# johannesulf/nautilus

Hardware: AMD Instinct MI355X
Metric: effective posterior samples/sec + |dlogZ| vs analytic, 50-dim Gaussian (higher is better)
Workload: dtype f64

## Files before the change

nautilus_amd/csrc/nb_eval_fast.hip:

```cpp
#include "nb_common.h"
#include "nb_launch.h"

#include <type_traits>

#include "nb_mlp.h"

namespace {

constexpr int FAST_MAX_GROUPS = 1024;

struct FastArgs {
  const double* blob;
  int sample;
  const nb_gd* x;
  const long long* idx;
  int m;
  int recentre;
  long long n;
  unsigned char* out_u8;
  double* out_f64;
  unsigned long long seed;
  unsigned long long offset;
  unsigned long long* counters;
  const FastGroup* groups;
  const int* totals;
  const int* dense;
  long long n_pad;
  int n_groups;
  int out_mode;
  unsigned char* st;
  int* first;
};

constexpr int FAST_B_DOUBLES =
    (NB_HT1 * NB_HT2 + NB_HT2 * NB_HT3 + NB_HT3) * NB_TILE;

typedef const void __attribute__((address_space(1))) * nbf_gptr;
typedef void __attribute__((address_space(3))) * nbf_lptr;

template <int DT, int T>
__device__ __forceinline__ void ell_eval_centre(
    const double* c, const double* tiles, int n_dim,
    const double (&xin)[T][4 * DT], int lane, int lg, double (&y)[T][4 * DT],
    double (&r2)[T]) {
  double d[T][4 * DT];
#pragma unroll
  for (int ks = 0; ks < 4 * DT; ++ks) {
    const double cv = c[4 * ks + lg];
#pragma unroll
    for (int t = 0; t < T; ++t) d[t][ks] = xin[t][ks] - cv;
  }
  double part[T];
#pragma unroll
  for (int t = 0; t < T; ++t) part[t] = 0.0;
  const int live = n_dim - 16 * (DT - 1);
  const bool small = DT > 1 && live >= 1 && live <= 4;
  const int lane4 = (lane >> 4) * 16 + (lane & 3);
#pragma unroll
  for (int ht = 0; ht < DT; ++ht) {
    if (ht == DT - 1 && small) {
      double r4[T];
#pragma unroll
      for (int t = 0; t < T; ++t) r4[t] = 0.0;
#pragma unroll
      for (int ks = 0; ks < 4 * (ht + 1) - 2; ++ks) {
        const int kt = ks >> 2, s = ks & 3;
        const double a =
            tiles[(ht * (ht + 1) / 2 + kt) * NB_TILE + s * 64 + lane4];
#pragma unroll
        for (int t = 0; t < T; ++t) r4[t] = MFMA4(a, d[t][ks], r4[t]);
      }
#pragma unroll
      for (int t = 0; t < T; ++t) {
        y[t][4 * ht] = r4[t];
        y[t][4 * ht + 1] = y[t][4 * ht + 2] = y[t][4 * ht + 3] = 0.0;
        part[t] += r4[t] * r4[t];
      }
    } else if (16 * ht < n_dim) {
      nb_d4 acc[T];
#pragma unroll
      for (int t = 0; t < T; ++t) acc[t] = nb_d4{0.0, 0.0, 0.0, 0.0};
#pragma unroll
      for (int ks = 0; ks < 4 * (ht + 1); ++ks) {
        const int kt = ks >> 2, s = ks & 3;
        const double a =
            tiles[(ht * (ht + 1) / 2 + kt) * NB_TILE + s * 64 + lane];
#pragma unroll
        for (int t = 0; t < T; ++t) acc[t] = MFMA(a, d[t][ks], acc[t]);
      }
#pragma unroll
      for (int t = 0; t < T; ++t)
#pragma unroll
        for (int r = 0; r < 4; ++r) {
          y[t][4 * ht + r] = acc[t][r];
          part[t] += acc[t][r] * acc[t][r];
        }
    } else {
#pragma unroll
      for (int t = 0; t < T; ++t)
#pragma unroll
        for (int r = 0; r < 4; ++r) y[t][4 * ht + r] = 0.0;
    }
  }
#pragma unroll
  for (int t = 0; t < T; ++t) r2[t] = lane_group_sum(part[t]);
}

template <int DT, int T>
__device__ __forceinline__ void load_points_raw(
    const nb_gd* __restrict__ x, const long long (&row_of)[T], int n_dim,
    int lane, double2 (&raw)[T][2 * DT]) {
  int lg = lane >> 4;
  asm volatile("" : "+v"(lg));
  asm volatile("" : "+s"(x));
  if ((n_dim & 1) == 0) {
#pragma unroll
    for (int t = 0; t < T; ++t) {
      const nb_gd* row = x + row_of[t] * n_dim;
#pragma unroll
      for (int j = 0; j < 2 * DT; ++j) {
        const int f = 8 * j + 2 * lg;
        raw[t][j] = *(const NB_G double2*)(row + (f < n_dim ? f : n_dim - 2));
      }
    }
  } else {
#pragma unroll
    for (int t = 0; t < T; ++t) {
      const nb_gd* row = x + row_of[t] * n_dim;
#pragma unroll
      for (int j = 0; j < 2 * DT; ++j) {
        const int f = 8 * j + 2 * lg;
        raw[t][j].x = row[f < n_dim ? f : n_dim - 1];
        raw[t][j].y = row[f + 1 < n_dim ? f + 1 : n_dim - 1];
      }
    }
  }
}

template <int DT, int T>
__device__ __forceinline__ void points_from_raw(
    const double2 (&raw)[T][2 * DT], const bool (&valid)[T], int n_dim,
    int lg, double (&xin)[T][4 * DT]) {
#pragma unroll
  for (int t = 0; t < T; ++t)
#pragma unroll
    for (int j = 0; j < 2 * DT; ++j) {
      const int f = 8 * j + 2 * lg;
      xin[t][2 * j] = (valid[t] && f < n_dim) ? raw[t][j].x : 0.0;
      xin[t][2 * j + 1] = (valid[t] && f + 1 < n_dim) ? raw[t][j].y : 0.0;
    }
}

constexpr int FAST_REGION = 38 * NB_TILE;

template <int DT, int KT1, bool BATCH>
__global__ void __launch_bounds__(512) nb_eval_fast_kernel(FastArgs a) {
  constexpr int T = 1, NW = 8, DP = 16 * DT;
  constexpr int KS1 = 4 * KT1;
  constexpr bool TWO = KT1 * NB_HT1 * NB_TILE > FAST_REGION;
  constexpr int KA = TWO ? (KT1 + 1) / 2 : KT1;
  constexpr int NT = DT * (DT + 1) / 2;
  constexpr int HEAD = 128;
  constexpr int TAIL = HEAD + NT * NB_TILE;
  constexpr int TC = (2 + 2 * DP + 127) / 128;
  constexpr int ELL_CHUNKS = 1 + 2 * NT + TC;
  static_assert(DP <= HEAD, "centre fits the head");
  static_assert(TAIL + TC * 128 <= FAST_REGION, "ellipsoid block fits a region");
  static_assert(KA * NB_HT1 * NB_TILE <= FAST_REGION, "layer-1 chunk fits");
  constexpr int NA_D = KA * NB_HT1 * NB_TILE;
  constexpr int NB1_D = (KT1 - KA) * NB_HT1 * NB_TILE;
  constexpr int NC_D = FAST_B_DOUBLES;
  extern __shared__ __attribute__((aligned(16))) double lds[];
  auto reg = [&](int i) __attribute__((always_inline)) {
    return lds + (i & 1) * FAST_REGION;
  };

  const int lane = threadIdx.x & 63;
  const int wave = __builtin_amdgcn_readfirstlane(threadIdx.x >> 6);
  const int lg = lane >> 4;
  const bool m_sample = a.sample != 0;
  const double* blob = a.blob;
  const int n_dim = (int)nb_hdr(blob, NB_H_NDIM);
  const int K = (int)nb_hdr(blob, NB_H_K);
  const bool use_cube = nb_hdr(blob, NB_H_USECUBE) != 0;
  const int ks1 = (n_dim + 1 + 3) >> 2;
  const long long net_stride = nb_hdr(blob, NB_H_NET_STRIDE);
  unsigned long long cnt_ell = 0, cnt_mlp = 0;
  long long sup = blockIdx.x;

  struct Pass {
    const double* nb;
    const double* shift;
    int E, b;
    long long base;
    int n_valid;
  };
  int* pp = (int*)(lds + 2 * FAST_REGION);
  long long n_super;
  if constexpr (BATCH) {
    if (wave == 0) {
      int run = 0;
      for (int g0 = 0; g0 < a.n_groups; g0 += 64) {
        const int g = g0 + lane;
        int v = g < a.n_groups ? (a.totals[g] + 127) >> 7 : 0;
#pragma unroll
        for (int d = 1; d < 64; d <<= 1) {
          const int u = __shfl_up(v, d);
          if (lane >= d) v += u;
        }
        if (g < a.n_groups) pp[g + 1] = run + v;
        run += __shfl(v, 63);
      }
      if (lane == 0) pp[0] = 0;
    }
    __syncthreads();
    n_super = pp[a.n_groups];
    if (sup >= n_super) return;
  } else {
    n_super = (a.n + 16 * NW * T - 1) / (16 * NW * T);
  }
  auto pass_of = [&](long long P) __attribute__((always_inline)) {
    Pass ps;
    if constexpr (BATCH) {
      const long long Pc = P < n_super ? P : n_super - 1;
      int lo = 0, hi = a.n_groups;
      while (hi - lo > 1) {
        const int mid = (lo + hi) >> 1;
        if (pp[mid] <= (int)Pc) lo = mid; else hi = mid;
      }
      const int g = __builtin_amdgcn_readfirstlane(lo);
      const FastGroup gd = a.groups[g];
      ps.nb = gd.nb;
      ps.shift = a.recentre != 0 ? gd.shift : nullptr;
      ps.E = gd.E;
      ps.b = gd.b;
      const int s0 = ((int)Pc - __builtin_amdgcn_readfirstlane(pp[g])) << 7;
      ps.base = (long long)g * a.n_pad + s0;
      const int left = a.totals[g] - s0;
      ps.n_valid = P < n_super ? (left < 128 ? left : 128) : 0;
    } else {
      ps.nb = blob + nb_hdr(blob, NB_H_OFF_NEURAL) +
              a.m * nb_hdr(blob, NB_H_NEURAL_STRIDE);
      ps.shift = (a.recentre != 0 && nb_hdr(blob, NB_H_OFF_SHIFT) != 0)
                     ? blob + nb_hdr(blob, NB_H_OFF_SHIFT) : nullptr;
      ps.E = (int)nb_hdr(blob, NB_H_E);
      ps.b = 0;
      ps.base = 0;
      ps.n_valid = 0;
    }
    return ps;
  };
  Pass cur_p = pass_of(sup);

  const double* dma_src = nullptr;
  double* dma_dst = nullptr;
  int dma_c = 0, dma_n = 0;
  bool dma_ell = false;
  auto dma_begin = [&](const double* src, double* dst, int n_doubles)
      __attribute__((always_inline)) {
    dma_src = src; dma_dst = dst; dma_c = wave; dma_n = n_doubles >> 7;
    dma_ell = false;
  };
  auto dma_begin_ell = [&](const double* nb_blk, double* dst)
      __attribute__((always_inline)) {
    dma_src = nb_blk; dma_dst = dst; dma_c = wave;
    dma_n = ELL_CHUNKS;
    dma_ell = true;
  };
  auto dma_one = [&]() __attribute__((always_inline)) {
    int s_off, d_off;
    if (!dma_ell) {
      s_off = d_off = dma_c * 128;
    } else if (dma_c < 1) {
      s_off = 2 + 2 * DP;
      d_off = 0;
    } else if (dma_c < 1 + 2 * NT) {
      const int p = (dma_c - 1) >> 1, half = (dma_c - 1) & 1;
      int ht = 0;
      while ((ht + 1) * (ht + 2) / 2 <= p) ++ht;
      const int kt = p - ht * (ht + 1) / 2;
      s_off = 2 + 3 * DP + (kt * DT + ht) * NB_TILE + half * 128;
      d_off = HEAD + p * NB_TILE + half * 128;
    } else {
      const int i = dma_c - 1 - 2 * NT;
      s_off = nb_ell_block_size(DT) + i * 128;
      d_off = TAIL + i * 128;
    }
    __builtin_amdgcn_global_load_lds(
        (nbf_gptr)(dma_src + s_off + 2 * lane),
        (nbf_lptr)(dma_dst + d_off), 16, 0, 0);
    dma_c += NW;
  };
  auto dma_tick = [&]() __attribute__((always_inline)) {
    if (dma_c < dma_n) dma_one();
  };
  auto dma_flush = [&]() __attribute__((always_inline)) {
    while (dma_c < dma_n) dma_one();
  };

  int q = 0;
  dma_begin_ell(cur_p.nb, reg(0));
  dma_flush();
  long long pt[T];
  bool valid[T];
  double2 xraw[T][2 * DT];
  auto row_of = [&](long long p) __attribute__((always_inline)) {
    return p < a.n ? (a.idx != nullptr ? a.idx[p] : p) : 0ll;
  };
  auto row_in = [&](const Pass& ps, int t) __attribute__((always_inline)) {
    const int slot = (wave * T + t) * 16 + (lane & 15);
    return (long long)a.dense[ps.base + (slot < ps.n_valid ? slot : 0)];
  };
  long long nrow[T];
#pragma unroll
  for (int t = 0; t < T; ++t) {
    pt[t] = ((sup * NW + wave) * T + t) * 16 + (lane & 15);
    valid[t] = pt[t] < a.n;
    if constexpr (BATCH) nrow[t] = row_in(cur_p, t);
    else nrow[t] = row_of(pt[t]);
  }
  load_points_raw<DT, T>(a.x, nrow, n_dim, lane, xraw);

  for (; sup < n_super; sup += gridDim.x) {
    const double* nb_m = cur_p.nb;
    const double* shift = cur_p.shift;
    const int E = cur_p.E;
    const double* nets = nb_m + nb_ell_block_size(DT) + 2 + 2 * DP;
    const Pass next_p = pass_of(sup + gridDim.x);
    int lgp = lg;
    asm volatile("" : "+v"(lgp));
    long long crow[T];
    dma_begin(nets, reg(q ^ 1), NA_D);
    dma_flush();
    asm volatile("s_waitcnt vmcnt(%0)" ::"n"((NA_D / 128 + NW - 1) / NW)
                 : "memory");
    __syncthreads();
    const double* blk = reg(q);
    const double thr = blk[TAIL];

    bool in_cube[T], acc_outer[T], want[T];
    double xin[T][4 * DT];
#pragma unroll
    for (int t = 0; t < T; ++t) {
      pt[t] = ((sup * NW + wave) * T + t) * 16 + (lane & 15);
      in_cube[t] = true;
      if constexpr (BATCH) {
        valid[t] = (wave * T + t) * 16 + (lane & 15) < cur_p.n_valid;
        crow[t] = nrow[t];
        nrow[t] = row_in(next_p, t);
      } else {
        valid[t] = pt[t] < a.n;
        nrow[t] = row_of((((sup + gridDim.x) * NW + wave) * T + t) * 16 +
                         (lane & 15));
      }
    }
    points_from_raw<DT, T>(xraw, valid, n_dim, lgp, xin);
    if (shift != nullptr) {
#pragma unroll
      for (int ks = 0; ks < 4 * DT; ++ks) {
        const double sv = shift[4 * ks + lgp];
        const bool on = shift[DP + 4 * ks + lgp] != 0.0;
#pragma unroll
        for (int t = 0; t < T; ++t) {
          const double v = xin[t][ks] + sv;
          xin[t][ks] = on ? v - floor(v) : xin[t][ks];
        }
      }
    }
    if (m_sample) {
      bool cbad[T];
#pragma unroll
      for (int t = 0; t < T; ++t) cbad[t] = false;
#pragma unroll
      for (int ks = 0; ks < 4 * DT; ++ks) {
        const int f = 8 * (ks >> 1) + 2 * lgp + (ks & 1);
        const bool boxed = use_cube && f < n_dim;
#pragma unroll
        for (int t = 0; t < T; ++t)
          cbad[t] |= boxed && !(xin[t][ks] >= 0.0 && xin[t][ks] < 1.0);
      }
#pragma unroll
      for (int t = 0; t < T; ++t) {
        in_cube[t] = !point_any(cbad[t], lane);
        acc_outer[t] = in_cube[t];
        want[t] = valid[t] && acc_outer[t];
      }
    } else {
#pragma unroll
      for (int t = 0; t < T; ++t) { acc_outer[t] = false; want[t] = valid[t]; }
    }

    double y[T][4 * DT], r2[T];
    bool box_bad[T], inside_e[T], need[T];
    ell_eval_centre<DT, T>(blk, blk + HEAD, n_dim, xin, lane, lgp, y, r2);
#pragma unroll
    for (int t = 0; t < T; ++t) box_bad[t] = false;
    bool wave_mlp = false;
#pragma unroll
    for (int t = 0; t < T; ++t) {
      inside_e[t] = !box_bad[t] && r2[t] < 1.0;
      need[t] = m_sample ? (want[t] && inside_e[t]) : valid[t];
      cnt_ell += __popcll(__ballot(want[t] && lg == 0));
      cnt_mlp += (unsigned long long)E * __popcll(__ballot(need[t] && lg == 0));
      wave_mlp |= need[t];
    }
    wave_mlp = __any(wave_mlp);

    double tin[T][KS1];
    {
      const double* r_mean = blk + TAIL + 2;
      const double* r_isc = r_mean + DP;
#pragma unroll
      for (int ks = 0; ks < KS1; ++ks) {
        const int f = 4 * ks + lgp;
        if (ks < 4 * DT) {
          const double mv = r_mean[f], sv = r_isc[f];
          const double pad = (f == n_dim) ? 1.0 : 0.0;
#pragma unroll
          for (int t = 0; t < T; ++t) {
            const double v = (y[t][ks] - mv) * sv;
            tin[t][ks] = (f < n_dim) ? v : pad;
          }
        } else {
#pragma unroll
          for (int t = 0; t < T; ++t) tin[t][ks] = (f == n_dim) ? 1.0 : 0.0;
        }
      }
    }
    asm volatile("s_waitcnt vmcnt(0)" ::: "memory");
    __syncthreads();
#pragma unroll
    for (int t = 0; t < T; ++t) asm volatile("" : "+v"(nrow[t]));

    double total[T];
#pragma unroll
    for (int t = 0; t < T; ++t) total[t] = 0.0;
    int cur = q ^ 1;

    auto stage_end = [&]() __attribute__((always_inline)) {
      dma_flush();
      asm volatile("s_waitcnt vmcnt(0)" ::: "memory");
      __syncthreads();
      cur ^= 1;
    };
    auto network = [&](int e, auto last_c) __attribute__((always_inline)) {
      constexpr bool LAST = decltype(last_c)::value;
      const double* w_e = nets + e * net_stride;
      double h1[T][4 * NB_HT1];
      if constexpr (TWO) {
        dma_begin(w_e + NA_D, reg(cur ^ 1), NB1_D);
        if (wave_mlp)
          fl_chunk<T, KS1, NB_HT1, 0, 4 * KA, 2>(reg(cur), ks1, tin, lane, h1,
                                                dma_tick);
        stage_end();
        dma_begin(w_e + NA_D + NB1_D, reg(cur ^ 1), NC_D);
        if (wave_mlp) {
          fl_chunk<T, KS1, NB_HT1, 4 * KA, KS1, 1>(reg(cur), ks1, tin, lane,
                                                  h1, dma_tick);
          fl_pad<T, NB_HT1, 25, 0>(h1, lane);
        }
        stage_end();
      } else {
        dma_begin(w_e + NA_D, reg(cur ^ 1), NC_D);
        if (wave_mlp) {
          fl_chunk<T, KS1, NB_HT1, 0, KS1, 1>(reg(cur), ks1, tin, lane, h1,
                                             dma_tick);
          fl_pad<T, NB_HT1, 25, 0>(h1, lane);
        }
        stage_end();
      }
      if constexpr (LAST) {
        load_points_raw<DT, T>(a.x, nrow, n_dim, lane, xraw);
        dma_begin_ell(next_p.nb, reg(cur ^ 1));
      } else {
        dma_begin(nets + (e + 1) * net_stride, reg(cur ^ 1), NA_D);
      }
      if (wave_mlp) {
        const double* w2 = reg(cur);
        const double* w3 = w2 + NB_HT1 * NB_HT2 * NB_TILE;
        const double* w4 = w3 + NB_HT2 * NB_HT3 * NB_TILE;
        double h2[T][4 * NB_HT2], h3[T][4 * NB_HT3], o[T][4];
        double a2[FlFirst<8, NB_HT2>::NA], a3[FlFirst<8, NB_HT3>::NA],
            a4[FlFirst<8, 1>::NA];
        fl_read_first<8, NB_HT2>(w2, lane, a2);
        fl_layer_from<T, 8, 26, 0, NB_HT2, true, 2, 1, 0>(
            w2, 26, h1, lane, h2, a2,
            [&]() __attribute__((always_inline)) {
              fl_read_first<8, NB_HT3>(w3, lane, a3);
            },
            dma_tick);
        fl_pad<T, NB_HT2, 12, 2>(h2, lane);
        fl_layer_from<T, 8, 13, 0, NB_HT3, true, 2, 2, 0>(
            w3, 13, h2, lane, h3, a3,
            [&]() __attribute__((always_inline)) {
              fl_read_first<8, 1>(w4, lane, a4);
            },
            dma_tick);
        fl_pad<T, NB_HT3, 5, 0>(h3, lane);
        fl_layer_from<T, 8, 6, 0, 1, true, 2, 5, 0>(
            w4, 6, h3, lane, o, a4, []() __attribute__((always_inline)) {},
            dma_tick);
#pragma unroll
        for (int t = 0; t < T; ++t) total[t] += o[t][0];
      }
      stage_end();
    };
    for (int e = 0; e + 1 < E; ++e) network(e, std::false_type{});
    network(E - 1, std::true_type{});
    q = cur;

#pragma unroll
    for (int t = 0; t < T; ++t) {
      const double score = __shfl(total[t], lane & 15) / (double)E;
      if constexpr (BATCH) {
        if (valid[t] && lg == 0 && score > thr) {
          a.st[crow[t]] = a.out_mode == 2 ? (unsigned char)3 : (unsigned char)2;
          if (a.out_mode == 1) atomicMin(&a.first[crow[t]], cur_p.b);
        }
      } else if (m_sample) {
        bool ok = inside_e[t];
        if (need[t]) ok = inside_e[t] && (score > thr);
        const unsigned char flags =
            (acc_outer[t] ? 1 : 0) | ((acc_outer[t] && ok) ? 2 : 0);
        if (valid[t] && lg == 0) a.out_u8[pt[t]] = flags;
      } else if (valid[t] && lg == 0) {
        a.out_f64[2 * pt[t]] = r2[t];
        a.out_f64[2 * pt[t] + 1] = score;
      }
    }
    cur_p = next_p;
  }
  if (a.counters != nullptr && lane == 0) {
    atomicAdd(&a.counters[1], cnt_ell);
    atomicAdd(&a.counters[2], cnt_mlp);
  }
}

template <int DT, int KT1, bool BATCH>
int launch_fast_impl(const FastArgs& a, hipStream_t stream) {
  const size_t lds = (size_t)2 * FAST_REGION * sizeof(double) +
                     (BATCH ? (FAST_MAX_GROUPS + 1) * sizeof(int) : 0);
  if (const int rc = nb_allow_lds<nb_eval_fast_kernel<DT, KT1, BATCH>>(lds))
    return rc;
  const long long n_super = (a.n + 127) / 128;
  long long blocks = n_super < 256 ? n_super : 256;
  hipLaunchKernelGGL((nb_eval_fast_kernel<DT, KT1, BATCH>),
                     dim3((unsigned)blocks), dim3(512), lds, stream, a);
  return NB_OK;
}

template <int DT, int KT1>
int launch_fast(const FastArgs& a, hipStream_t stream) {
  return a.groups != nullptr ? launch_fast_impl<DT, KT1, true>(a, stream)
                             : launch_fast_impl<DT, KT1, false>(a, stream);
}

}

bool nb_eval_fast_eligible(int n_dim, int K, int M, int E, bool sample) {
  if (n_dim > 128 || M < 1 || E < 1) return false;
  return !sample || (K <= 1 && M == 1);
}

static int dispatch_fast(const FastArgs& a, int n_dim, hipStream_t stream) {
  const int kt1 = (n_dim + 1 + 15) / 16;
  const int rc = nb_tile_dispatch((n_dim + 15) / 16, [&](auto dt) {
    constexpr int DT = decltype(dt)::value;
    return kt1 == DT ? launch_fast<DT, DT>(a, stream)
                     : launch_fast<DT, DT + 1>(a, stream);
  });
  if (rc != NB_OK) return rc;
  NB_HIP_CHECK(hipGetLastError());
  return NB_OK;
}

int nb_launch_eval_fast(const double* blob_dev, int n_dim, bool sample, int m,
                        int recentre, const double* x, const long long* idx,
                        long long n,
                        unsigned char* out_u8, double* out_f64,
                        unsigned long long seed, unsigned long long offset,
                        hipStream_t stream) {
  if (n <= 0) return NB_OK;
  FastArgs a = {};
  a.blob = blob_dev; a.sample = sample ? 1 : 0; a.x = (const nb_gd*)x; a.n = n;
  a.idx = idx; a.m = m; a.recentre = recentre;
  a.out_u8 = out_u8; a.out_f64 = out_f64; a.seed = seed; a.offset = offset;
  a.counters = nb_eval_counters();
  return dispatch_fast(a, n_dim, stream);
}

int nb_launch_eval_fast_batch(const double* blob0_dev, int n_dim, int recentre,
                              const double* x, const void* groups_dev,
                              int n_groups, const int* totals_dev,
                              const int* dense_dev, long long n_pad,
                              long long n_upper, int out_mode,
                              unsigned char* st, int* first,
                              hipStream_t stream) {
  if (n_upper <= 0 || n_groups <= 0) return NB_OK;
  if (n_groups > FAST_MAX_GROUPS) {
    nb_set_error("nb_launch_eval_fast_batch: %d groups (limit %d)", n_groups,
                 FAST_MAX_GROUPS);
    return NB_ERR_ARG;
  }
  FastArgs a = {};
  a.blob = blob0_dev; a.sample = 0; a.x = (const nb_gd*)x;
  a.n = n_upper + 128ll * n_groups;
  a.recentre = recentre;
  a.counters = nb_eval_counters();
  a.groups = (const FastGroup*)groups_dev; a.n_groups = n_groups;
  a.totals = totals_dev; a.dense = dense_dev; a.n_pad = n_pad;
  a.out_mode = out_mode; a.st = st; a.first = first;
  return dispatch_fast(a, n_dim, stream);
}
```

Before: 2.595 million.

## Keep ellipsoid block resident in LDS and reuse layer-1 region across iterations

For non-batched small-dimension configurations, the kernel now sizes LDS so the ellipsoid block lives in its own resident area, and the first-layer weights stay in a fixed region. This removes the per-iteration re-DMA of the ellipsoid block and the layer-1 chunk plus one barrier per super-iteration. Prologue and epilogue are factored into lambdas, and an optional compile-time stagger mode (off by default) lets half the waves precompute the next prologue. The catch is a larger LDS footprint, which may reduce occupancy, and more code complexity.

```diff
diff --git a/nautilus_amd/csrc/nb_eval_fast.hip b/nautilus_amd/csrc/nb_eval_fast.hip
--- a/nautilus_amd/csrc/nb_eval_fast.hip
+++ b/nautilus_amd/csrc/nb_eval_fast.hip
@@ -106,10 +106,11 @@
   for (int t = 0; t < T; ++t) r2[t] = lane_group_sum(part[t]);
 }
 
-template <int DT, int T>
+template <int DT, int T, int NR>
 __device__ __forceinline__ void load_points_raw(
     const nb_gd* __restrict__ x, const long long (&row_of)[T], int n_dim,
-    int lane, double2 (&raw)[T][2 * DT]) {
+    int lane, double2 (&raw)[T][NR]) {
+  static_assert(NR >= 2 * DT, "a row's slots fit");
   int lg = lane >> 4;
   asm volatile("" : "+v"(lg));
   asm volatile("" : "+s"(x));
@@ -137,9 +138,9 @@
   }
 }
 
-template <int DT, int T>
+template <int DT, int T, int NR>
 __device__ __forceinline__ void points_from_raw(
-    const double2 (&raw)[T][2 * DT], const bool (&valid)[T], int n_dim,
+    const double2 (&raw)[T][NR], const bool (&valid)[T], int n_dim,
     int lg, double (&xin)[T][4 * DT]) {
 #pragma unroll
   for (int t = 0; t < T; ++t)
@@ -152,12 +153,43 @@
 }
 
 constexpr int FAST_REGION = 38 * NB_TILE;
+constexpr size_t FAST_LDS_BUDGET = 160 * 1024;
+#ifndef NB_FAST_STAGGER
+#define NB_FAST_STAGGER 0
+#endif
+constexpr bool FAST_STAGGER = NB_FAST_STAGGER != 0;
+
+constexpr int fast_block_doubles(int DT) {
+  return 128 + DT * (DT + 1) / 2 * NB_TILE + (2 + 32 * DT + 127) / 128 * 128;
+}
+constexpr bool fast_two(int KT1) {
+  return KT1 * NB_HT1 * NB_TILE > FAST_REGION;
+}
+constexpr size_t fast_resident_bytes(int DT, int KT1) {
+  return ((size_t)(KT1 * NB_HT1 + 38) * NB_TILE + fast_block_doubles(DT)) *
+         sizeof(double);
+}
+constexpr bool fast_resident(int DT, int KT1, bool BATCH) {
+  return !BATCH && !fast_two(KT1) &&
+         fast_resident_bytes(DT, KT1) <= FAST_LDS_BUDGET;
+}
+constexpr size_t fast_lds_bytes(int DT, int KT1, bool BATCH) {
+  return fast_resident(DT, KT1, BATCH)
+             ? fast_resident_bytes(DT, KT1)
+             : (size_t)2 * FAST_REGION * sizeof(double) +
+                   (BATCH ? (FAST_MAX_GROUPS + 1) * sizeof(int) : 0);
+}
 
 template <int DT, int KT1, bool BATCH>
 __global__ void __launch_bounds__(512) nb_eval_fast_kernel(FastArgs a) {
   constexpr int T = 1, NW = 8, DP = 16 * DT;
   constexpr int KS1 = 4 * KT1;
-  constexpr bool TWO = KT1 * NB_HT1 * NB_TILE > FAST_REGION;
+  constexpr bool TWO = fast_two(KT1);
+  constexpr bool RES = fast_resident(DT, KT1, BATCH);
+  static_assert(fast_lds_bytes(DT, KT1, BATCH) <= FAST_LDS_BUDGET,
+                "regions, ellipsoid block and pass table fit the LDS");
+  static_assert(RES == (!BATCH && (DT <= 3 || (DT == 4 && KT1 == 4))),
+                "resident form: every DT <= 3 and <4, 4>");
   constexpr int KA = TWO ? (KT1 + 1) / 2 : KT1;
   constexpr int NT = DT * (DT + 1) / 2;
   constexpr int HEAD = 128;
@@ -165,15 +197,18 @@
   constexpr int TC = (2 + 2 * DP + 127) / 128;
   constexpr int ELL_CHUNKS = 1 + 2 * NT + TC;
   static_assert(DP <= HEAD, "centre fits the head");
+  static_assert(TAIL + TC * 128 == fast_block_doubles(DT), "block size");
   static_assert(TAIL + TC * 128 <= FAST_REGION, "ellipsoid block fits a region");
   static_assert(KA * NB_HT1 * NB_TILE <= FAST_REGION, "layer-1 chunk fits");
   constexpr int NA_D = KA * NB_HT1 * NB_TILE;
   constexpr int NB1_D = (KT1 - KA) * NB_HT1 * NB_TILE;
   constexpr int NC_D = FAST_B_DOUBLES;
   extern __shared__ __attribute__((aligned(16))) double lds[];
+  constexpr int REG0_D = RES ? KT1 * NB_HT1 * NB_TILE : FAST_REGION;
   auto reg = [&](int i) __attribute__((always_inline)) {
-    return lds + (i & 1) * FAST_REGION;
-  };
+    return lds + (i & 1) * REG0_D;
+  };
+  double* const blk_res = lds + REG0_D + FAST_REGION;
 
   const int lane = threadIdx.x & 63;
   const int wave = __builtin_amdgcn_readfirstlane(threadIdx.x >> 6);
@@ -298,12 +333,151 @@
     while (dma_c < dma_n) dma_one();
   };
 
+  constexpr int NR = RES ? 2 * KT1 : 2 * DT;
+  auto slot_of = [&](long long P, int t) __attribute__((always_inline)) {
+    int l = lane;
+    asm volatile("" : "+v"(l));
+    return ((P * NW + wave) * T + t) * 16 + (l & 15);
+  };
+  enum : unsigned { PS_VALID = 1, PS_OUTER = 2, PS_INSIDE = 4, PS_NEED = 8 };
+  struct PState {
+    unsigned bits[T];
+    bool wave_mlp;
+    double r2[T];
+  };
+  auto prologue = [&](const double* blk, const double* shift, int E,
+                      const double2 (&raw)[T][NR], const bool (&valid)[T],
+                      PState& s, double (&tin)[T][KS1])
+      __attribute__((always_inline)) {
+    int lgp = lg;
+    asm volatile("" : "+v"(lgp));
+    int lanep = lane;
+    asm volatile("" : "+v"(lanep));
+    bool in_cube[T], want[T], acc_outer[T];
+    double xin[T][4 * DT];
+    points_from_raw<DT, T>(raw, valid, n_dim, lgp, xin);
+    if (shift != nullptr) {
+#pragma unroll
+      for (int ks = 0; ks < 4 * DT; ++ks) {
+        const double sv = shift[4 * ks + lgp];
+        const bool on = shift[DP + 4 * ks + lgp] != 0.0;
+#pragma unroll
+        for (int t = 0; t < T; ++t) {
+          const double v = xin[t][ks] + sv;
+          xin[t][ks] = on ? v - floor(v) : xin[t][ks];
+        }
+      }
+    }
+    if (m_sample) {
+      bool cbad[T];
+#pragma unroll
+      for (int t = 0; t < T; ++t) cbad[t] = false;
+#pragma unroll
+      for (int ks = 0; ks < 4 * DT; ++ks) {
+        const int f = 8 * (ks >> 1) + 2 * lgp + (ks & 1);
+        const bool boxed = use_cube && f < n_dim;
+#pragma unroll
+        for (int t = 0; t < T; ++t)
+          cbad[t] |= boxed && !(xin[t][ks] >= 0.0 && xin[t][ks] < 1.0);
+      }
+#pragma unroll
+      for (int t = 0; t < T; ++t) {
+        in_cube[t] = !point_any(cbad[t], lanep);
+        acc_outer[t] = in_cube[t];
+        want[t] = valid[t] && acc_outer[t];
+      }
+    } else {
+#pragma unroll
+      for (int t = 0; t < T; ++t) {
+        acc_outer[t] = false;
+        want[t] = valid[t];
+      }
+    }
+
+    double y[T][4 * DT];
+    ell_eval_centre<DT, T>(blk, blk + HEAD, n_dim, xin, lanep, lgp, y, s.r2);
+    bool wave_mlp = false;
+#pragma unroll
+    for (int t = 0; t < T; ++t) {
+      const bool inside_e = s.r2[t] < 1.0;
+      const bool need = m_sample ? (want[t] && inside_e) : valid[t];
+      cnt_ell += __popcll(__ballot(want[t] && lg == 0));
+      cnt_mlp += (unsigned long long)E * __popcll(__ballot(need && lg == 0));
+      wave_mlp |= need;
+      s.bits[t] = (valid[t] ? PS_VALID : 0u) | (acc_outer[t] ? PS_OUTER : 0u) |
+                  (inside_e ? PS_INSIDE : 0u) | (need ? PS_NEED : 0u);
+    }
+    s.wave_mlp = __any(wave_mlp);
+
+    const double* r_mean = blk + TAIL + 2;
+    const double* r_isc = r_mean + DP;
+#pragma unroll
+    for (int ks = 0; ks < KS1; ++ks) {
+      const int f = 4 * ks + lgp;
+      if (ks < 4 * DT) {
+        const double mv = r_mean[f], sv = r_isc[f];
+        const double pad = (f == n_dim) ? 1.0 : 0.0;
+#pragma unroll
+        for (int t = 0; t < T; ++t) {
+          const double v = (y[t][ks] - mv) * sv;
+          tin[t][ks] = (f < n_dim) ? v : pad;
+        }
+      } else {
+#pragma unroll
+        for (int t = 0; t < T; ++t) tin[t][ks] = (f == n_dim) ? 1.0 : 0.0;
+      }
+    }
+  };
+  auto epilogue = [&](const PState& s, long long P, const double (&total)[T],
+                      double thr, int E, const long long (&crow)[T], int b)
+      __attribute__((always_inline)) {
+#pragma unroll
+    for (int t = 0; t < T; ++t) {
+      const double score = __shfl(total[t], lane & 15) / (double)E;
+      const bool valid = (s.bits[t] & PS_VALID) != 0;
+      const bool acc_outer = (s.bits[t] & PS_OUTER) != 0;
+      const bool inside_e = (s.bits[t] & PS_INSIDE) != 0;
+      const bool need = (s.bits[t] & PS_NEED) != 0;
+      const long long pt = slot_of(P, t);
+      if constexpr (BATCH) {
+        if (valid && lg == 0 && score > thr) {
+          a.st[crow[t]] = a.out_mode == 2 ? (unsigned char)3 : (unsigned char)2;
+          if (a.out_mode == 1) atomicMin(&a.first[crow[t]], b);
+        }
+      } else if (m_sample) {
+        bool ok = inside_e;
+        if (need) ok = inside_e && (score > thr);
+        const unsigned char flags =
+            (acc_outer ? 1 : 0) | ((acc_outer && ok) ? 2 : 0);
+        if (valid && lg == 0) a.out_u8[pt] = flags;
+      } else if (valid && lg == 0) {
+        a.out_f64[2 * pt] = s.r2[t];
+        a.out_f64[2 * pt + 1] = score;
+      }
+    }
+  };
+
   int q = 0;
-  dma_begin_ell(cur_p.nb, reg(0));
-  dma_flush();
-  long long pt[T];
-  bool valid[T];
-  double2 xraw[T][2 * DT];
+  double2 xraw[T][NR];
+  auto tin_park = [&](const double (&tin)[T][KS1])
+      __attribute__((always_inline)) {
+#pragma unroll
+    for (int t = 0; t < T; ++t)
+#pragma unroll
+      for (int j = 0; j < 2 * KT1; ++j) {
+        xraw[t][j].x = tin[t][2 * j];
+        xraw[t][j].y = tin[t][2 * j + 1];
+      }
+  };
+  auto tin_unpark = [&](double (&tin)[T][KS1]) __attribute__((always_inline)) {
+#pragma unroll
+    for (int t = 0; t < T; ++t)
+#pragma unroll
+      for (int j = 0; j < 2 * KT1; ++j) {
+        tin[t][2 * j] = xraw[t][j].x;
+        tin[t][2 * j + 1] = xraw[t][j].y;
+      }
+  };
   auto row_of = [&](long long p) __attribute__((always_inline)) {
     return p < a.n ? (a.idx != nullptr ? a.idx[p] : p) : 0ll;
   };
@@ -312,130 +486,87 @@
     return (long long)a.dense[ps.base + (slot < ps.n_valid ? slot : 0)];
   };
   long long nrow[T];
-#pragma unroll
-  for (int t = 0; t < T; ++t) {
-    pt[t] = ((sup * NW + wave) * T + t) * 16 + (lane & 15);
-    valid[t] = pt[t] < a.n;
-    if constexpr (BATCH) nrow[t] = row_in(cur_p, t);
-    else nrow[t] = row_of(pt[t]);
+  auto nrow_arrived = [&]() __attribute__((always_inline)) {
+#pragma unroll
+    for (int t = 0; t < T; ++t) asm volatile("" : "+v"(nrow[t]));
+  };
+  PState st, st_n;
+  double tin[T][KS1];
+  if constexpr (RES) {
+#pragma unroll
+    for (int t = 0; t < T; ++t) nrow[t] = row_of(slot_of(sup, t));
+    load_points_raw<DT, T>(a.x, nrow, n_dim, lane, xraw);
+#pragma unroll
+    for (int t = 0; t < T; ++t) nrow[t] = row_of(slot_of(sup + gridDim.x, t));
+    dma_begin_ell(cur_p.nb, blk_res);
+    dma_flush();
+    dma_begin(cur_p.nb + nb_ell_block_size(DT) + 2 + 2 * DP, reg(0), NA_D);
+    dma_flush();
+    asm volatile("s_waitcnt vmcnt(0)" ::: "memory");
+    __syncthreads();
+    nrow_arrived();
+  } else {
+    dma_begin_ell(cur_p.nb, reg(0));
+    dma_flush();
+#pragma unroll
+    for (int t = 0; t < T; ++t) {
+      if constexpr (BATCH) nrow[t] = row_in(cur_p, t);
+      else nrow[t] = row_of(slot_of(sup, t));
+    }
+    load_points_raw<DT, T>(a.x, nrow, n_dim, lane, xraw);
   }
-  load_points_raw<DT, T>(a.x, nrow, n_dim, lane, xraw);
-
-  for (; sup < n_super; sup += gridDim.x) {
+
+  for (bool first = true; sup < n_super; sup += gridDim.x, first = false) {
     const double* nb_m = cur_p.nb;
     const double* shift = cur_p.shift;
     const int E = cur_p.E;
     const double* nets = nb_m + nb_ell_block_size(DT) + 2 + 2 * DP;
     const Pass next_p = pass_of(sup + gridDim.x);
-    int lgp = lg;
-    asm volatile("" : "+v"(lgp));
     long long crow[T];
-    dma_begin(nets, reg(q ^ 1), NA_D);
-    dma_flush();
-    asm volatile("s_waitcnt vmcnt(%0)" ::"n"((NA_D / 128 + NW - 1) / NW)
-                 : "memory");
-    __syncthreads();
-    const double* blk = reg(q);
-    const double thr = blk[TAIL];
-
-    bool in_cube[T], acc_outer[T], want[T];
-    double xin[T][4 * DT];
-#pragma unroll
-    for (int t = 0; t < T; ++t) {
-      pt[t] = ((sup * NW + wave) * T + t) * 16 + (lane & 15);
-      in_cube[t] = true;
-      if constexpr (BATCH) {
-        valid[t] = (wave * T + t) * 16 + (lane & 15) < cur_p.n_valid;
-        crow[t] = nrow[t];
-        nrow[t] = row_in(next_p, t);
+    double thr = 0.0;
+    const bool more = sup + gridDim.x < n_super;
+    const bool early = FAST_STAGGER && wave < 4;
+    if constexpr (RES) {
+      if (first || !early) {
+        bool valid[T];
+#pragma unroll
+        for (int t = 0; t < T; ++t) valid[t] = slot_of(sup, t) < a.n;
+        prologue(blk_res, shift, E, xraw, valid, st, tin);
       } else {
-        valid[t] = pt[t] < a.n;
-        nrow[t] = row_of((((sup + gridDim.x) * NW + wave) * T + t) * 16 +
-                         (lane & 15));
-      }
-    }
-    points_from_raw<DT, T>(xraw, valid, n_dim, lgp, xin);
-    if (shift != nullptr) {
-#pragma unroll
-      for (int ks = 0; ks < 4 * DT; ++ks) {
-        const double sv = shift[4 * ks + lgp];
-        const bool on = shift[DP + 4 * ks + lgp] != 0.0;
-#pragma unroll
-        for (int t = 0; t < T; ++t) {
-          const double v = xin[t][ks] + sv;
-          xin[t][ks] = on ? v - floor(v) : xin[t][ks];
-        }
-      }
-    }
-    if (m_sample) {
-      bool cbad[T];
-#pragma unroll
-      for (int t = 0; t < T; ++t) cbad[t] = false;
-#pragma unroll
-      for (int ks = 0; ks < 4 * DT; ++ks) {
-        const int f = 8 * (ks >> 1) + 2 * lgp + (ks & 1);
-        const bool boxed = use_cube && f < n_dim;
-#pragma unroll
-        for (int t = 0; t < T; ++t)
-          cbad[t] |= boxed && !(xin[t][ks] >= 0.0 && xin[t][ks] < 1.0);
-      }
+        st = st_n;
+        tin_unpark(tin);
+      }
+    } else {
+      dma_begin(nets, reg(q ^ 1), NA_D);
+      dma_flush();
+      asm volatile("s_waitcnt vmcnt(%0)" ::"n"((NA_D / 128 + NW - 1) / NW)
+                   : "memory");
+      __syncthreads();
+      const double* blk = reg(q);
+      thr = blk[TAIL];
+      bool valid[T];
 #pragma unroll
       for (int t = 0; t < T; ++t) {
-        in_cube[t] = !point_any(cbad[t], lane);
-        acc_outer[t] = in_cube[t];
-        want[t] = valid[t] && acc_outer[t];
-      }
-    } else {
-#pragma unroll
-      for (int t = 0; t < T; ++t) { acc_outer[t] = false; want[t] = valid[t]; }
-    }
-
-    double y[T][4 * DT], r2[T];
-    bool box_bad[T], inside_e[T], need[T];
-    ell_eval_centre<DT, T>(blk, blk + HEAD, n_dim, xin, lane, lgp, y, r2);
-#pragma unroll
-    for (int t = 0; t < T; ++t) box_bad[t] = false;
-    bool wave_mlp = false;
-#pragma unroll
-    for (int t = 0; t < T; ++t) {
-      inside_e[t] = !box_bad[t] && r2[t] < 1.0;
-      need[t] = m_sample ? (want[t] && inside_e[t]) : valid[t];
-      cnt_ell += __popcll(__ballot(want[t] && lg == 0));
-      cnt_mlp += (unsigned long long)E * __popcll(__ballot(need[t] && lg == 0));
-      wave_mlp |= need[t];
-    }
-    wave_mlp = __any(wave_mlp);
-
-    double tin[T][KS1];
-    {
-      const double* r_mean = blk + TAIL + 2;
-      const double* r_isc = r_mean + DP;
-#pragma unroll
-      for (int ks = 0; ks < KS1; ++ks) {
-        const int f = 4 * ks + lgp;
-        if (ks < 4 * DT) {
-          const double mv = r_mean[f], sv = r_isc[f];
-          const double pad = (f == n_dim) ? 1.0 : 0.0;
-#pragma unroll
-          for (int t = 0; t < T; ++t) {
-            const double v = (y[t][ks] - mv) * sv;
-            tin[t][ks] = (f < n_dim) ? v : pad;
-          }
+        if constexpr (BATCH) {
+          valid[t] = (wave * T + t) * 16 + (lane & 15) < cur_p.n_valid;
+          crow[t] = nrow[t];
+          nrow[t] = row_in(next_p, t);
         } else {
-#pragma unroll
-          for (int t = 0; t < T; ++t) tin[t][ks] = (f == n_dim) ? 1.0 : 0.0;
-        }
-      }
-    }
-    asm volatile("s_waitcnt vmcnt(0)" ::: "memory");
-    __syncthreads();
-#pragma unroll
-    for (int t = 0; t < T; ++t) asm volatile("" : "+v"(nrow[t]));
+          valid[t] = slot_of(sup, t) < a.n;
+          nrow[t] = row_of(slot_of(sup + gridDim.x, t));
+        }
+      }
+      prologue(blk, shift, E, xraw, valid, st, tin);
+      asm volatile("s_waitcnt vmcnt(0)" ::: "memory");
+      __syncthreads();
+      nrow_arrived();
+    }
 
     double total[T];
 #pragma unroll
     for (int t = 0; t < T; ++t) total[t] = 0.0;
-    int cur = q ^ 1;
+    int cur = RES ? 0 : q ^ 1;
+    const bool wave_mlp = st.wave_mlp;
 
     auto stage_end = [&]() __attribute__((always_inline)) {
       dma_flush();
@@ -446,30 +577,51 @@
     auto network = [&](int e, auto last_c) __attribute__((always_inline)) {
       constexpr bool LAST = decltype(last_c)::value;
       const double* w_e = nets + e * net_stride;
+      int lanes = lane;
+      asm volatile("" : "+v"(lanes));
       double h1[T][4 * NB_HT1];
       if constexpr (TWO) {
         dma_begin(w_e + NA_D, reg(cur ^ 1), NB1_D);
         if (wave_mlp)
-          fl_chunk<T, KS1, NB_HT1, 0, 4 * KA, 2>(reg(cur), ks1, tin, lane, h1,
+          fl_chunk<T, KS1, NB_HT1, 0, 4 * KA, 2>(reg(cur), ks1, tin, lanes, h1,
                                                 dma_tick);
         stage_end();
         dma_begin(w_e + NA_D + NB1_D, reg(cur ^ 1), NC_D);
         if (wave_mlp) {
-          fl_chunk<T, KS1, NB_HT1, 4 * KA, KS1, 1>(reg(cur), ks1, tin, lane,
+          fl_chunk<T, KS1, NB_HT1, 4 * KA, KS1, 1>(reg(cur), ks1, tin, lanes,
                                                   h1, dma_tick);
-          fl_pad<T, NB_HT1, 25, 0>(h1, lane);
+          fl_pad<T, NB_HT1, 25, 0>(h1, lanes);
         }
         stage_end();
       } else {
+        if constexpr (RES && LAST) {
+          if (more && early)
+            load_points_raw<DT, T>(a.x, nrow, n_dim, lane, xraw);
+        }
         dma_begin(w_e + NA_D, reg(cur ^ 1), NC_D);
         if (wave_mlp) {
-          fl_chunk<T, KS1, NB_HT1, 0, KS1, 1>(reg(cur), ks1, tin, lane, h1,
+          fl_chunk<T, KS1, NB_HT1, 0, KS1, 1>(reg(cur), ks1, tin, lanes, h1,
                                              dma_tick);
-          fl_pad<T, NB_HT1, 25, 0>(h1, lane);
+          fl_pad<T, NB_HT1, 25, 0>(h1, lanes);
         }
         stage_end();
       }
-      if constexpr (LAST) {
+      if constexpr (LAST && RES) {
+        if (more) {
+          if (early) {
+            bool valid[T];
+#pragma unroll
+            for (int t = 0; t < T; ++t)
+              valid[t] = slot_of(sup + gridDim.x, t) < a.n;
+            double tin_n[T][KS1];
+            prologue(blk_res, shift, E, xraw, valid, st_n, tin_n);
+            tin_park(tin_n);
+          } else {
+            load_points_raw<DT, T>(a.x, nrow, n_dim, lane, xraw);
+          }
+        }
+        dma_begin(nets, reg(cur ^ 1), NA_D);
+      } else if constexpr (LAST) {
         load_points_raw<DT, T>(a.x, nrow, n_dim, lane, xraw);
         dma_begin_ell(next_p.nb, reg(cur ^ 1));
       } else {
@@ -482,52 +634,40 @@
         double h2[T][4 * NB_HT2], h3[T][4 * NB_HT3], o[T][4];
         double a2[FlFirst<8, NB_HT2>::NA], a3[FlFirst<8, NB_HT3>::NA],
             a4[FlFirst<8, 1>::NA];
-        fl_read_first<8, NB_HT2>(w2, lane, a2);
+        fl_read_first<8, NB_HT2>(w2, lanes, a2);
         fl_layer_from<T, 8, 26, 0, NB_HT2, true, 2, 1, 0>(
-            w2, 26, h1, lane, h2, a2,
+            w2, 26, h1, lanes, h2, a2,
             [&]() __attribute__((always_inline)) {
-              fl_read_first<8, NB_HT3>(w3, lane, a3);
+              fl_read_first<8, NB_HT3>(w3, lanes, a3);
             },
             dma_tick);
-        fl_pad<T, NB_HT2, 12, 2>(h2, lane);
+        fl_pad<T, NB_HT2, 12, 2>(h2, lanes);
         fl_layer_from<T, 8, 13, 0, NB_HT3, true, 2, 2, 0>(
-            w3, 13, h2, lane, h3, a3,
+            w3, 13, h2, lanes, h3, a3,
             [&]() __attribute__((always_inline)) {
-              fl_read_first<8, 1>(w4, lane, a4);
+              fl_read_first<8, 1>(w4, lanes, a4);
             },
             dma_tick);
-        fl_pad<T, NB_HT3, 5, 0>(h3, lane);
+        fl_pad<T, NB_HT3, 5, 0>(h3, lanes);
         fl_layer_from<T, 8, 6, 0, 1, true, 2, 5, 0>(
-            w4, 6, h3, lane, o, a4, []() __attribute__((always_inline)) {},
+            w4, 6, h3, lanes, o, a4, []() __attribute__((always_inline)) {},
             dma_tick);
 #pragma unroll
         for (int t = 0; t < T; ++t) total[t] += o[t][0];
       }
+      if constexpr (LAST && RES) {
+#pragma unroll
+        for (int t = 0; t < T; ++t)
+          nrow[t] = row_of(slot_of(sup + 2 * (long long)gridDim.x, t));
+      }
       stage_end();
+      if constexpr (LAST && RES) nrow_arrived();
     };
     for (int e = 0; e + 1 < E; ++e) network(e, std::false_type{});
     network(E - 1, std::true_type{});
-    q = cur;
-
-#pragma unroll
-    for (int t = 0; t < T; ++t) {
-      const double score = __shfl(total[t], lane & 15) / (double)E;
-      if constexpr (BATCH) {
-        if (valid[t] && lg == 0 && score > thr) {
-          a.st[crow[t]] = a.out_mode == 2 ? (unsigned char)3 : (unsigned char)2;
-          if (a.out_mode == 1) atomicMin(&a.first[crow[t]], cur_p.b);
-        }
-      } else if (m_sample) {
-        bool ok = inside_e[t];
-        if (need[t]) ok = inside_e[t] && (score > thr);
-        const unsigned char flags =
-            (acc_outer[t] ? 1 : 0) | ((acc_outer[t] && ok) ? 2 : 0);
-        if (valid[t] && lg == 0) a.out_u8[pt[t]] = flags;
-      } else if (valid[t] && lg == 0) {
-        a.out_f64[2 * pt[t]] = r2[t];
-        a.out_f64[2 * pt[t] + 1] = score;
-      }
-    }
+    if constexpr (!RES) q = cur;
+
+    epilogue(st, sup, total, RES ? blk_res[TAIL] : thr, E, crow, cur_p.b);
     cur_p = next_p;
   }
   if (a.counters != nullptr && lane == 0) {
@@ -538,8 +678,7 @@
 
 template <int DT, int KT1, bool BATCH>
 int launch_fast_impl(const FastArgs& a, hipStream_t stream) {
-  const size_t lds = (size_t)2 * FAST_REGION * sizeof(double) +
-                     (BATCH ? (FAST_MAX_GROUPS + 1) * sizeof(int) : 0);
+  const size_t lds = fast_lds_bytes(DT, KT1, BATCH);
   if (const int rc = nb_allow_lds<nb_eval_fast_kernel<DT, KT1, BATCH>>(lds))
     return rc;
   const long long n_super = (a.n + 127) / 128;
```

Measured after the change: 2.495 million. 3.9% lower.
